# zhykoties/Multi-Head-Recommendation-with-Human-Priors

Hardware: AMD Instinct MI355X
Metric: user-sequences/sec/node (HSTU Pixel8M, seqlen 200) (higher is better)
Workload: dtype bf16; 1 GPU; cfg1: HSTU Pixel8M-shaped train step, L=200 P=8 D=256 8 layers x 8 heads, 4 prior heads, N=453938 items, 8192 negatives/pool, B=128/GPU, loss=prior, bf16-mixed, fused AdamW over all parameters (item table: lazy replay of gradient-free steps, flushed inside the timed region); step replayed from a hipGraph; encoder on packed rows (the loader's row capacity, one step graph per capacity); global_batch=128, seq_len=200, parallelism=dp1

## Files before the change

### include/mhr.h

```cpp
#ifndef MHR_H
#define MHR_H

#include <stdint.h>

#ifdef __cplusplus
extern "C" {
#endif

#define MHR_F32 0
#define MHR_BF16 1

#define MHR_OK 0
#define MHR_EINVAL (-1)
#define MHR_ELAUNCH (-2)

const char* mhr_last_error(void);
int mhr_abi_version(void);


int mhr_bad_id_count(int64_t* host_count, int reset);

int mhr_embedding_gather_fwd(const float* table, int64_t n_rows, int dim,
                             const int64_t* ids, int64_t n_ids,
                             void* out, int out_dtype,
                             const float* pos_table, int seq_len, int window_len,
                             void* x_out, int x_dtype, int64_t n_x_ids, void* stream);

int mhr_embedding_gather_step(const float* table, int64_t n_rows, int dim, const int64_t* ids, int64_t n_ids,
                              int64_t n_item_ids, float* rows_out, const float* pos_table, int seq_len, int window_len,
                              float* x_out, void* neg_out, float* neg_norms, const int32_t* row_of, const int32_t* src_of,
                              int capacity, void* stream);

int mhr_embedding_scatter_add_bwd(const void* grad_rows, int grad_dtype, const int64_t* ids, int64_t n_ids,
                                  float* grad_table, int64_t n_rows, int dim, void* stream);

int mhr_sparse_rows_segment_sum(const int64_t* sorted_ids, const int64_t* perm, int64_t n_ids,
                                const void* grad_a, int a_dtype, int64_t n_a,
                                const void* grad_b, int b_dtype, int64_t n_b,
                                const float* x_grad, int seq_len, int window_len, const int32_t* x_row_of,
                                float* out_rows, int32_t* row_slot, int64_t n_rows, int dim, void* stream);

int mhr_pos_grad_packed(const float* d_x, const int32_t* row_of, int B, int L, int dim, float* out, void* stream);
int mhr_window_rows_add_packed(const float* rows, int64_t n_rows, int window_len, int seq_len, const float* d_x,
                               const int32_t* row_of, int dim, float* out, void* stream);

int mhr_adam_rows(float* w, float* m, float* v, int64_t n_rows, int dim,
                  const float* grad_rows, int32_t* row_slot, float grad_scale,
                  float lr, float beta1, float beta2, float eps, float weight_decay, int step, void* stream);

int mhr_adam_flat(float* w, const float* g, float* m, float* v, int64_t n, float grad_scale,
                  float lr, float beta1, float beta2, float eps, float weight_decay, int step, void* w_bf16,
                  const float* hist, int hist_len, const int64_t* step_dev, void* stream);
int mhr_adam_consts(float lr, float beta1, float beta2, float eps, float weight_decay, int step, float* out4);
int mhr_adam_rows_lazy(float* w, float* m, float* v, int64_t n_rows, int dim, const int64_t* ids, int64_t n_ids,
                       const float* grad_rows, int32_t* row_slot, int32_t* last_step, const float* hist,
                       int hist_len, int step, float grad_scale, float beta1, float beta2, float eps, int mode,
                       const int64_t* step_dev, void* stream);

int mhr_sum_rows_into(const void* x_bf16, int64_t rows, int64_t cols, float* out, void* stream);
int mhr_sum_rows_f32_into(const float* x, int64_t rows, int64_t cols, float* out, void* stream);
int mhr_sum_rows_many(const int64_t* ptrs, int n, int64_t rows, int64_t cols, void* stream);


int mhr_layernorm_fwd(const void* x, int x_dtype, void* y, int y_dtype, float* mean, float* rstd,
                      int64_t rows, int dim, float eps, void* stream);
int mhr_layernorm_bwd(const void* dy, int dy_dtype, const void* x, int x_dtype, const float* mean, const float* rstd,
                      void* dx, int dx_dtype, int accumulate, int64_t rows, int dim, void* stream);
int mhr_add_cast(const float* x, const void* y_bf16, float* out, void* out_bf16, int64_t n, void* stream);

int mhr_add_layernorm_fwd(const float* x, const void* y_bf16, float* x_out, void* xn_bf16, float* mean, float* rstd,
                          int64_t rows, int dim, float eps, const int32_t* first_row, int seq_len, void* stream);
int mhr_add_layernorm_bwd(const void* d_xn_bf16, const float* x_out, const float* mean, const float* rstd,
                          const float* d_xout, float* dx, void* dy_bf16, int64_t rows, int dim,
                          const int32_t* first_row, int seq_len, void* stream);

int mhr_ln_gate_fwd(const void* u_base, int64_t u_stride, const void* a, int dtype, void* o, int o_dtype,
                    float* mean, float* rstd, int64_t rows, int dim, float eps,
                    float dropout_p, uint64_t seed, const int64_t* step_seed,
                    const int32_t* first_row, int seq_len, void* stream);
int mhr_ln_gate_bwd(const void* d_o, int do_dtype, const void* u_base, int64_t u_stride, const void* a, int dtype,
                    const float* mean, const float* rstd, void* du_base, int64_t du_stride, void* da,
                    int64_t rows, int dim, float dropout_p, uint64_t seed, const int64_t* step_seed,
                    const int32_t* first_row, int seq_len, void* stream);

int mhr_l2norm_rows(const void* x, int x_dtype, void* y, int y_dtype, float* norms, int64_t rows, int dim, void* stream);
int mhr_l2norm_rows_bwd(const float* dy, const float* x, const float* norms, float* dx, int64_t rows, int dim, void* stream);
int mhr_l2norm_rows_indexed_bwd(const float* dy, const float* table, int64_t n_src_rows, const int64_t* ids, const float* norms,
                                float* dx, int64_t rows, int dim, void* stream);

int mhr_hstu_attn_fwd(const void* q, const void* k, const void* v, int64_t row_stride,
                      const uint8_t* key_valid, void* out,
                      void* act_q, void* act_k, void* act_v, int64_t act_stride,
                      int B, int L, int n_heads, int head_dim, int apply_silu, void* stream);
int mhr_hstu_attn_bwd(const void* q_pre, const void* k_pre, const void* v_pre, int64_t row_stride,
                      const void* act_q, const void* act_k, const void* act_v, int64_t act_stride,
                      const uint8_t* key_valid, const void* d_out,
                      void* dq, void* dk, void* dv, int64_t d_stride,
                      int B, int L, int n_heads, int head_dim, int apply_silu, void* stream);

int mhr_rows_gemm_supported(int M, int N, int K, int w_is_kn);
int mhr_rows_gemm(const void* a, int64_t lda, const void* w, int64_t ldw, int w_is_kn, const void* bias,
                  void* c, int64_t ldc, int M, int N, int K, void* stream);

int mhr_attn_seq_layout(const uint8_t* key_valid, int B, int L, int32_t* first_block, int32_t* seq_order,
                        int32_t* first_row , void* stream);
int mhr_hstu_attn_fwd_seq(const void* q, const void* k, const void* v, int64_t row_stride,
                          const uint8_t* key_valid, void* out,
                          void* act_q, void* act_k, void* act_v, int64_t act_stride,
                          int B, int L, int n_heads, int head_dim, int apply_silu,
                          const int32_t* first_block, const int32_t* seq_order, const int32_t* cu_rows, int n_rows_total,
                          void* stream);
int mhr_hstu_attn_bwd_seq(const void* q_pre, const void* k_pre, const void* v_pre, int64_t row_stride,
                          const void* act_q, const void* act_k, const void* act_v, int64_t act_stride,
                          const uint8_t* key_valid, const void* d_out,
                          void* dq, void* dk, void* dv, int64_t d_stride,
                          int B, int L, int n_heads, int head_dim, int apply_silu,
                          const int32_t* first_block, const int32_t* seq_order, const int32_t* cu_rows, int n_rows_total,
                          void* stream);

int mhr_seq_pack_maps(const uint8_t* key_valid, int B, int L, int capacity, int32_t* cu_rows, int32_t* src_of, int32_t* row_of,
                      int32_t* overflow, void* stream);
int mhr_seq_pack_maps_guarded(const uint8_t* key_valid, int B, int L, int capacity, int32_t* cu_rows, int32_t* src_of,
                              int32_t* row_of, int32_t* overflow, int32_t* guard, void* stream);
int mhr_rows_gather_masked(const void* src, int dtype, const int32_t* idx, void* out, int64_t n_out, int dim, void* stream);


int mhr_rmsnorm_fwd(const float* x, const void* res_bf16, const float* weight, float* x_out, void* y_bf16, float* rstd,
                    int64_t rows, int dim, float eps, void* stream);
int mhr_rmsnorm_bwd_parts(int64_t rows);
int mhr_rmsnorm_bwd(const void* dy_bf16, const float* x_out, const float* weight, const float* rstd, const float* d_xout,
                    float* dx, void* dres_bf16, float* dw_part, int64_t rows, int dim, void* stream);

int mhr_swiglu_fwd(const void* gate_up_bf16, void* act_bf16, int64_t rows, int ffn, void* stream);
int mhr_swiglu_bwd(const void* gate_up_bf16, const void* d_act_bf16, void* d_gate_up_bf16, int64_t rows, int ffn, void* stream);

int mhr_rope_inplace(void* x_bf16, int64_t row_stride, const int32_t* positions, const float* cos_table,
                     const float* sin_table, int64_t n_tokens, int seq_len, int n_heads, int head_dim, int max_pos,
                     int inverse, void* stream);

int mhr_softmax_attn_fwd(const void* q, const void* k, const void* v, int64_t row_stride, const int32_t* cu_seqlens,
                         const uint8_t* key_valid, void* out, float* lse, int n_seqs, int max_len, int n_heads,
                         int n_kv_heads, int head_dim, float scale, void* stream);
int mhr_softmax_attn_bwd(const void* q, const void* k, const void* v, int64_t row_stride, const int32_t* cu_seqlens,
                         const uint8_t* key_valid, const void* out, const void* d_out, const float* lse, void* dq,
                         int64_t dq_stride, void* dk, void* dv, int64_t dkv_stride, int n_seqs, int max_len, int n_heads,
                         int n_kv_heads, int head_dim, float scale, void* stream);

int mhr_token_compact(const uint8_t* mask, const int32_t* q_all, const int32_t* p_all, const int32_t* o_all,
                      int n_groups, int n_slots, int tok_cap, int32_t* q_idx, int32_t* p_idx, int32_t* o_idx,
                      int32_t* n_tok, int32_t* scratch, int32_t* tok_of_slot, const int32_t* row_of, int seq_len,
                      int n_heads, int head_stride, void* stream);

int mhr_heads_residual_fwd(const float* x, const void* z_bf16, float* out, int64_t n_tok, int seq_len, int n_heads,
                           int dim, void* stream);
int mhr_heads_residual_bwd(const float* d_out, const void* z_bf16, void* dz_bf16, float* dx, int64_t n_tok,
                           int seq_len, int n_heads, int dim, void* stream);

int mhr_row_maps(const int32_t* q_idx, const int32_t* n_tok_dev, int n_groups, int tok_cap, int row_cap,
                 int32_t* row_q, int32_t* row_first, int32_t* tok2row, int32_t* n_row, int32_t* scratch, void* stream);

int mhr_nce_log_counters(const int32_t* n_valid, const int32_t* rank, const int32_t* o_idx, const int32_t* n_tok_dev,
                         int group, int tok_cap, const int32_t* ks_host, int n_k, uint64_t* scratch8, float* out, void* stream);

int mhr_loss_reduce(const float* bucket_sum, const float* bucket_cnt, const float* weight, int n_groups, int n_buckets,
                    int n_segments, float* total, float* out, void* stream);
int mhr_loss_reduce_bwd(const float* d_total, const float* bucket_cnt, const float* weight, int n, float* w_out, void* stream);

int mhr_nce_fwd(const void* q_rows, const int32_t* q_idx, const void* p_rows, const int32_t* p_idx, int io_dtype,
                const void* negs, int n_neg, int dim, int n_groups, const int32_t* n_tok_dev, int tok_cap,
                const float* logit_scale_dev, float thres,
                float* sum_out, int32_t* n_valid, int32_t* rank,
                void* qn_out, void* pn_out, uint32_t* supp_out, float* q_inv, float* p_inv, float* s_pos,
                int log_group, float* u_out, int64_t n_p_rows, uint32_t* fix_words, const int32_t* fix_row_list,
                const int32_t* fix_n_rows, int32_t* fix_slot_of_row, void* stream);
int mhr_nce_finalize(const float* sum, const float* s_pos, int n_groups, const int32_t* n_tok_dev, int tok_cap,
                     const float* logit_scale_dev, float* loss, float* lse, int32_t* n_valid,
                     const int32_t* bucket_idx, int n_buckets, float* bucket_sum, float* bucket_cnt, void* stream);
int mhr_nce_bwd_tokens(const void* qn, const void* pn, const float* u, int dim, int n_groups,
                       const int32_t* n_tok_dev, int tok_cap, const float* logit_scale_dev,
                       const float* lse, const float* w, const float* q_inv, const float* p_inv, const float* s_pos,
                       const int32_t* q_idx, const int32_t* p_idx,
                       float* dq_rows, float* dp_rows, float* d_logit_scale, float* lw_out,
                       const int32_t* w_bucket, int n_buckets, int64_t* dq_fix, int64_t* dp_fix,
                       float* dls_part, void* stream);
int mhr_nce_bwd_negs(const void* qn, const void* negs, const uint32_t* supp, int n_neg, int dim, int n_groups,
// ... 145 lines not shown
```

### multi-head-recommendation-with-human-priors_amd/code/REC/model/hstu_functional.py

```python
import os
from collections import OrderedDict

import torch
from torch.autograd import Function

from mhr_amd import ops

_SPLITK_MAX = int(os.environ.get("MHR_SPLITK_MAX", "16"))
_SUM_KERNEL = os.environ.get("MHR_SUM_KERNEL", "1") != "0"


class LayerNormFn(Function):

    @staticmethod
    def forward(ctx, x, eps, out=None):
        y, mean, rstd = ops.layernorm_fwd(x, torch.bfloat16, eps, out=out)
        ctx.save_for_backward(x, mean, rstd)
        return y

    @staticmethod
    def backward(ctx, dy):
        x, mean, rstd = ctx.saved_tensors
        return ops.layernorm_bwd(dy.contiguous(), x, mean, rstd, dx_dtype=torch.float32), None, None

# ... 31 lines not shown
    @staticmethod
    def backward(ctx, d_xout, d_xn):
        x_out, mean, rstd = ctx.saved_tensors
        if d_xout is None:
            d_xout = torch.zeros_like(x_out)
        if d_xn is None:
            d_xn = torch.zeros(x_out.shape, dtype=torch.bfloat16, device=x_out.device)
        dx, dy = ops.add_layernorm_bwd(d_xn.contiguous(), x_out, mean, rstd, d_xout.contiguous().float(), dy_out=ctx.dy_out,
                                       dead=ctx.dead)
        return dx, dy, None, None, None, None


class AddCastFn(Function):

    @staticmethod
    def forward(ctx, x, y, dy_out=None):
        ctx.dy_out = dy_out
        return ops.add_cast(x.contiguous(), y.contiguous())

    @staticmethod
    def backward(ctx, d_out, d_out16):
        if d_out is None and d_out16 is None:
            return None, None, None
        if d_out16 is None:
            return d_out, d_out.to(torch.bfloat16), None
        if d_out is None:
            return d_out16.float(), d_out16, None
        return ops.add_cast(d_out.contiguous(), d_out16.contiguous(), out16=ctx.dy_out) + (None,)


class WeightGradStack:

    def __init__(self, opt, uvqk_params, o_params, R, D, device):
        L = len(uvqk_params)
        self.opt, self.L, self.R, self.D = opt, L, R, D
        self.params = {"uvqk": list(uvqk_params), "o": list(o_params)}
        bf = dict(dtype=torch.bfloat16, device=device)
        self.xn, self.dh = torch.empty(L, R, D, **bf), torch.empty(L, R, 4 * D, **bf)
        self.o, self.dy = torch.empty(L, R, D, **bf), torch.empty(L, R, D, **bf)
        self.seen = {"uvqk": set(), "o": set()}
        opt.defer(self.flush)

    def operands(self, kind, layer, x, dy):
        xs, ds = (self.xn, self.dh) if kind == "uvqk" else (self.o, self.dy)
        if x.data_ptr() != xs[layer].data_ptr():
            xs[layer].copy_(x.reshape(xs[layer].shape))
        if dy.data_ptr() != ds[layer].data_ptr():
            ds[layer].copy_(dy.reshape(ds[layer].shape))
        self.seen[kind].add(layer)

    @staticmethod
    def _splits(R, prefer):
        return next((s for s in prefer if R % s == 0 and R // s >= 256), 1)

    def flush(self):
        n = {k: len(v) for k, v in self.seen.items()}
        if n["uvqk"] == 0 and n["o"] == 0:
            return
        if n["uvqk"] != self.L or n["o"] != self.L:
            raise RuntimeError(f"WeightGradStack: {n} of {self.L} layers handed their operands over")
        L, R, D = self.L, self.R, self.D
        S1 = self._splits(R, (8, 4, 2))
        w1 = torch.bmm(self.xn.view(L * S1, R // S1, D).transpose(1, 2), self.dh.view(L * S1, R // S1, 4 * D))
        S2 = self._splits(R, (16, 8, 4, 2))
        w2 = torch.bmm(self.dy.view(L * S2, R // S2, D).transpose(1, 2), self.o.view(L * S2, R // S2, D))
        for l in range(L):
            self.opt.queue_rows_sum(w1[l * S1:(l + 1) * S1].view(S1, -1), self.params["uvqk"][l].grad)
            self.opt.queue_rows_sum(w2[l * S2:(l + 1) * S2].view(S2, -1), self.params["o"][l].grad)
        self.seen = {"uvqk": set(), "o": set()}


ROWS_GEMM = os.environ.get("MHR_ROWS_GEMM", "1") != "0"
ROWS_GEMM_MIN_M = int(os.environ.get("MHR_ROWS_GEMM_MIN_M", "8192"))


def _rows_gemm_pays(x, w_kn):
    M, K = x.shape
    N = w_kn.shape[1]
    return (K == 256 and N >= 1024 and M >= ROWS_GEMM_MIN_M and x.dtype == torch.bfloat16 and w_kn.dtype == torch.bfloat16
            and x.stride(1) == 1 and w_kn.is_contiguous() and x.stride(0) % 8 == 0 and x.data_ptr() % 16 == 0 and w_kn.data_ptr() % 16 == 0
            and ops.rows_gemm_supported(M, N, K, True))


class SplitKLinearFn(Function):

    @staticmethod
    def forward(ctx, x, w, b, w_is_nk, w_bf16, defer=None):
        ctx.defer = defer
        if w_bf16 is None:
            sh = getattr(w, "_mhr_bf16", None)
            w_bf16 = sh if (sh is not None and w._version == w._mhr_ver) else None
        wb = w.to(torch.bfloat16) if w_bf16 is None else w_bf16
        bb = None
        if b is not None:
            sh = getattr(b, "_mhr_bf16", None)
            bb = sh if (sh is not None and b._version == b._mhr_ver) else b.to(torch.bfloat16)
        if w_is_nk:
            y = torch.nn.functional.linear(x, wb, bb)
        elif ROWS_GEMM and _rows_gemm_pays(x, wb):
            y = ops.rows_gemm(x, wb, None, w_is_kn=True)
        else:
            y = x @ wb
        ctx.save_for_backward(x, wb)
        ctx.w_is_nk, ctx.has_bias = w_is_nk, b is not None
        ctx.w_leaf = w if getattr(w, "_mhr_direct_grad", False) and w.grad is not None else None
        ctx.b_leaf = b if (b is not None and getattr(b, "_mhr_direct_grad", False) and b.grad is not None) else None
        return y

    @staticmethod
    def _into(leaf, parts):
        g = leaf.grad
        if _SUM_KERNEL and parts.dtype == torch.bfloat16 and parts.is_contiguous() and g.is_contiguous() and g.numel() % 8 == 0:
            ops.sum_rows_into(parts, g)
        else:
            g.add_(torch.sum(parts, 0, dtype=torch.float32).view_as(g))

    @staticmethod
    def backward(ctx, dy):
        x, wb = ctx.saved_tensors
        dy = dy.contiguous()
        dx = dy @ wb if ctx.w_is_nk else dy @ wb.t()
        R = x.shape[0]
        if ctx.defer is not None and ctx.w_leaf is not None:
            stack, kind, layer = ctx.defer
            stack.operands(kind, layer, x, dy)
            if ctx.has_bias and ctx.b_leaf is not None:
                bopt = getattr(ctx.b_leaf, "_mhr_opt", None)
                if not (bopt is not None and bopt.queue_bias_sum(dy, ctx.b_leaf)):
                    SplitKLinearFn._into(ctx.b_leaf, dy)
                return dx, None, None, None, None, None
            return dx, None, (torch.sum(dy, 0, dtype=torch.float32) if ctx.has_bias else None), None, None, None
        tiles = -(-wb.shape[0] // 256) * -(-wb.shape[1] // 256)
        s_max = min(max(1, 256 // tiles), _SPLITK_MAX)
        S = next((s for s in (64, 32, 16, 8, 4, 2) if s <= s_max and R % s == 0 and R // s >= 256), 1)
        xs, dys = x.view(S, R // S, -1), dy.view(S, R // S, -1)
        opt = getattr(ctx.w_leaf, "_mhr_opt", None) if ctx.w_leaf is not None else None
        slot = opt.partial_view(ctx.w_leaf, S) if (opt is not None and S > 1 and _SUM_KERNEL) else None
        if ctx.w_is_nk:
            dw = torch.bmm(dys.transpose(1, 2), xs, out=slot) if slot is not None else torch.bmm(dys.transpose(1, 2), xs)
        else:
            dw = torch.bmm(xs.transpose(1, 2), dys, out=slot) if slot is not None else torch.bmm(xs.transpose(1, 2), dys)
        if slot is not None:
            dw = None
        elif ctx.w_leaf is not None:
            SplitKLinearFn._into(ctx.w_leaf, dw)
            dw = None
        else:
            dw = torch.sum(dw, 0, dtype=torch.float32) if S > 1 else dw[0].float()
        db = None
        if ctx.has_bias:
            if ctx.b_leaf is not None:
                bopt = getattr(ctx.b_leaf, "_mhr_opt", None)
                if not (bopt is not None and _SUM_KERNEL and bopt.queue_bias_sum(dy, ctx.b_leaf)):
                    SplitKLinearFn._into(ctx.b_leaf, dy)
            else:
                db = torch.sum(dy, 0, dtype=torch.float32)
        return dx, dw, db, None, None, None


class FusedHeadsLinearFn(Function):

    @staticmethod
    def forward(ctx, x, w16, b16, gw, gb):
        ctx.save_for_backward(x, w16)
        ctx.gw, ctx.gb = gw, gb
        return torch.nn.functional.linear(x, w16, b16)

    @staticmethod
    def backward(ctx, dy):
        x, w16 = ctx.saved_tensors
        dy = dy.contiguous()
        dx = dy @ w16
        R = x.shape[0]
        tiles = -(-w16.shape[0] // 256) * -(-w16.shape[1] // 256)
        s_max = min(max(1, 256 // tiles), _SPLITK_MAX)
        S = next((s for s in (64, 32, 16, 8, 4, 2) if s <= s_max and R % s == 0 and R // s >= 256), 1)
        dw = torch.bmm(dy.view(S, R // S, -1).transpose(1, 2), x.view(S, R // S, -1))
        ops.sum_rows_into(dw, ctx.gw)
        ops.sum_rows_into(dy, ctx.gb)
        return dx, None, None, None, None


class HeadsResidualFn(Function):

    @staticmethod
    def forward(ctx, x, z, B, L, H):
        ctx.save_for_backward(z)
        ctx.cfg = (B, L, H)
        return ops.heads_residual_fwd(x.contiguous(), z.contiguous(), B, L, H)

    @staticmethod
    def backward(ctx, d_out):
        (z,) = ctx.saved_tensors
        B, L, H = ctx.cfg
        dz, dx = ops.heads_residual_bwd(d_out.contiguous().float(), z, B, L, H)
        return dx, dz, None, None, None


class FusedParamLinearFn(Function):

    @staticmethod
    def forward(ctx, x, w16, gview, leaf):
        ctx.save_for_backward(x, w16)
        ctx.gview, ctx.leaf = gview, leaf
        return torch.nn.functional.linear(x, w16)

    @staticmethod
    def backward(ctx, dy):
        from mhr_amd import optim
        x, w16 = ctx.saved_tensors
        dy = dy.contiguous()
        dx = dy @ w16
        dw = torch.mm(dy.t(), x, out_dtype=torch.float32)
        if getattr(ctx.leaf, "_mhr_epoch_f", -1) != optim.GRAD_EPOCH:
            ctx.leaf._mhr_epoch_f = optim.GRAD_EPOCH
            ctx.gview.copy_(dw)
        else:
            ctx.gview.add_(dw)
        return dx, None, None, None


class MoveRowsFn(Function):

    @staticmethod
    def forward(ctx, x, fwd_idx, bwd_idx):
        ctx.bwd_idx = bwd_idx
        return ops.rows_gather_masked(x.contiguous(), fwd_idx)

    @staticmethod
    def backward(ctx, dy):
        return ops.rows_gather_masked(dy.contiguous(), ctx.bwd_idx), None, None


class HSTUCoreFn(Function):

    @staticmethod
    def forward(ctx, h, key_valid, B, L, n_heads, head_dim, eps, dropout_p, seed, seed_dev=None, o_out=None, dh_out=None):
        D = n_heads * head_dim
        layout = getattr(key_valid, "_mhr_layout", None)
        a, _ = ops.hstu_attn_fwd(h, key_valid, B, L, n_heads, head_dim, apply_silu=True, save_act=False, layout=layout)
        dead = (layout[2], L) if (ops.DEAD_ROWS and layout is not None and len(layout) > 2 and layout[2] is not None
                                  and getattr(key_valid, "_mhr_dead_ok", True)) else None
        o, mean, rstd = ops.ln_gate_fwd(h, a, D, torch.bfloat16, eps, dropout_p, seed, seed_dev, out=o_out, dead=dead)
        ctx.dh_out = dh_out
        ctx.save_for_backward(h, key_valid, a, mean, rstd)
        ctx.cfg = (B, L, n_heads, head_dim, dropout_p, seed, seed_dev)
        ctx.layout, ctx.dead = layout, dead
        return o

    @staticmethod
    def backward(ctx, d_o):
        h, key_valid, a, mean, rstd = ctx.saved_tensors
        B, L, n_heads, head_dim, dropout_p, seed, seed_dev = ctx.cfg
        D = n_heads * head_dim
        dh = torch.empty_like(h) if ctx.dh_out is None else ctx.dh_out.view(h.shape)
# ... 294 lines not shown
```

### multi-head-recommendation-with-human-priors_amd/csrc/rows_gemm.hip

```cpp
#include <algorithm>

#include "stream_gemm.h"

namespace {

typedef unsigned u32x2_t __attribute__((ext_vector_type(2)));

#ifdef RGX_STAMP
__device__ unsigned long long g_rg_stamps[4096 * 4];
#define RG_STAMP(k)                                                                     \
  {                                                                                     \
    __builtin_amdgcn_sched_barrier(0);                                                  \
    unsigned long long t_;                                                              \
    asm volatile("s_memtime %0\n\ts_waitcnt lgkmcnt(0)" : "=s"(t_)::"memory");          \
    __builtin_amdgcn_sched_barrier(0);                                                  \
    if (threadIdx.x == 0 && blockIdx.x < 4096) g_rg_stamps[blockIdx.x * 4 + (k)] = t_;  \
  }
#define RG_PHASE(k)                                                                     \
  {                                                                                     \
    __builtin_amdgcn_sched_barrier(0);                                                  \
    unsigned long long t_;                                                              \
    asm volatile("s_memtime %0\n\ts_waitcnt lgkmcnt(0)" : "=s"(t_)::"memory");          \
    __builtin_amdgcn_sched_barrier(0);                                                  \
    pacc_[k] += t_ - ph_;                                                               \
// ... 127 lines not shown
    } else {
      dp.template piece<k>(tiles + slot * T::BYTES, reinterpret_cast<const char*>(A) + (int64_t)tn * T::BYTES);
    }
  };
  auto dma_tile = [&](auto slot_c, int tn) {
    auto f = [&](auto k_c) { dma_piece(slot_c, k_c, tn); };
    sg::static_for<P::PW>(f);
  };
  sg::RowAddr<NKS> ra;
  ra.init(la, tiles);

  const int n_lane = n_wave + 8 * half;
  const bool full_cols = n_wave + 64 <= N;

  const int n_loc = t1 - t0, t_last = t1 - 1;
  dma_tile(std::integral_constant<int, 0>{}, t0);
  dma_tile(std::integral_constant<int, 1>{}, min(t0 + 1, t_last));
#ifdef RGX_STAMP
  unsigned long long ph_ = 0, pacc_[8] = {0, 0, 0, 0, 0, 0, 0, 0};
  RG_PHASE(7)
#endif
  sg::u32x4 o[RF][2];
  auto store_piece = [&](auto idx_c, int ts, bool all) {
    constexpr int idx = decltype(idx_c)::value, f = idx >> 1, gp = idx & 1;
    bf16_t* p = C + (int64_t)(ts * 32 + r) * ldc + n_lane + f * 32 + gp * 16;
    if (all || (ts * 32 + r < M && n_lane + f * 32 + gp * 16 < N)) *reinterpret_cast<sg::u32x4*>(p) = o[f][gp];
  };
  constexpr int NOPS = P::PW + 4;
  sg::ring_loop<3>(n_loc, [&](auto slot_c, int i) {
    constexpr int cur = decltype(slot_c)::value, nxt = (cur + 2) % 3;
    const int t = t0 + i;
    RG_PHASE(0)
    if (i > 2 && full_cols) sg::wait_vmcnt<P::PW + 8>();
    else if (i == 2 && full_cols) sg::wait_vmcnt<P::PW + 4>();
    else sg::wait_vmcnt<P::PW>();
    sg::ring_barrier();
    RG_PHASE(1)
    f32x16 acc[RF];
#pragma unroll
    for (int f = 0; f < RF; ++f) {
      if constexpr (HAS_BIAS) acc[f] = acc0[f];
      else acc[f] = sg::zero16();
    }
    const int t_dma = min(t + 2, t_last);
    const bool st_all = full_cols;
    mma_tile_gaps<NKS, RF, cur * T::BYTES>(ra, frag, acc, [&](auto ks_c) {
      constexpr int ks = decltype(ks_c)::value;
      auto op = [&](auto j_c) {
        constexpr int jj = decltype(j_c)::value;
        if constexpr (jj * NKS / NOPS == ks) {
          if constexpr (jj < P::PW) dma_piece(std::integral_constant<int, nxt>{}, j_c, t_dma);
          else if (i > 0) store_piece(std::integral_constant<int, jj - P::PW>{}, t - 1, st_all);
        }
      };
      sg::static_for<NOPS>(op);
    });
    RG_PHASE(3)
#pragma unroll
    for (int f = 0; f < RF; ++f) {
#pragma unroll
      for (int gp = 0; gp < 2; ++gp) {
        const int gx = 8 * gp, gy = 8 * gp + 4;
        const uint32_t x0 = sg::cvt_pk_bf16(acc[f][gx + 0], acc[f][gx + 1]), x1 = sg::cvt_pk_bf16(acc[f][gx + 2], acc[f][gx + 3]);
        const uint32_t y0 = sg::cvt_pk_bf16(acc[f][gy + 0], acc[f][gy + 1]), y1 = sg::cvt_pk_bf16(acc[f][gy + 2], acc[f][gy + 3]);
        const u32x2_t s0 = __builtin_amdgcn_permlane32_swap(x0, y0, false, false);
        const u32x2_t s1 = __builtin_amdgcn_permlane32_swap(x1, y1, false, false);
        o[f][gp] = sg::u32x4{s0.x, s1.x, s0.y, s1.y};
      }
    }
    RG_PHASE(4)
  });
  {
    const bool all = full_cols && t_last * 32 + 32 <= M;
    auto st = [&](auto idx_c) { store_piece(idx_c, t_last, all); };
    sg::static_for<4>(st);
  }
  RG_STAMP(2)
#ifdef RGX_STAMP
  if (threadIdx.x == 0 && blockIdx.x == 37)
    for (int k = 0; k < 7; ++k) g_rg_stamps[4096 * 4 - 8 + k] += pacc_[k];
#endif
  sg::wait_vmcnt<0>();
  RG_STAMP(3)
}

}

#ifdef RGX_STAMP
extern "C" int mhr_debug_read_rg_stamps(unsigned long long* host, int n) {
  return (int)hipMemcpyFromSymbol(host, HIP_SYMBOL(g_rg_stamps), (size_t)n * sizeof(unsigned long long));
}
#endif

extern "C" int mhr_rows_gemm_supported(int M, int N, int K, int w_is_kn) {
  return (K == 64 || K == 128 || K == 256) && N > 0 && N % (w_is_kn ? 256 : 8) == 0 && M > 0;
}

extern "C" int mhr_rows_gemm(const void* a, int64_t lda, const void* w, int64_t ldw, int w_is_kn, const void* bias, void* c,
                             int64_t ldc, int M, int N, int K, void* stream) {
  MHR_REQUIRE(a && w && c, "rows_gemm: null pointer");
  MHR_REQUIRE(mhr_rows_gemm_supported(M, N, K, w_is_kn),
              "rows_gemm: M=%d N=%d K=%d unsupported (K in {64, 128, 256}; N a multiple of 8, of 256 with W stored [K, N])", M, N, K);
  MHR_REQUIRE(lda >= K && ldw >= (w_is_kn ? N : K) && ldc >= N && lda % 8 == 0 && ldw % 8 == 0 && ldc % 8 == 0,
              "rows_gemm: leading dimensions must cover the rows and be multiples of 8 elements");
  MHR_REQUIRE(((uintptr_t)a | (uintptr_t)w | (uintptr_t)c) % 16 == 0, "rows_gemm: operands must be 16-byte aligned");
  const int n_tiles = (M + 31) / 32;
  const int n_cg = (N + 255) / 256;
  int n_streams = (512 / n_cg) & ~7;
  while (n_streams > 8 && n_tiles / n_streams < 3) n_streams -= 8;
  if (n_streams < 8) n_streams = 8;
  const bool strided = lda != K || M % 32 != 0;
  const int nks = K / 16;
  size_t lds = 4 * (size_t)(32 * K * 2);
  if (w_is_kn) lds = std::max(lds, (size_t)std::min(K / 32, 4) * 16384);
  hipStream_t s = (hipStream_t)stream;
#define L____(NKS, ST, HB, KN)                                                                                            \
  hipLaunchKernelGGL((rows_gemm_kernel<NKS, ST, HB, KN>), dim3(n_cg * n_streams), dim3(256), lds, s, (const bf16_t*)a, lda, \
                     (const bf16_t*)w, ldw, (const bf16_t*)bias, (bf16_t*)c, ldc, M, N, n_tiles, n_cg, n_streams)
#define L___(NKS, ST, HB)                    \
  if (w_is_kn) { L____(NKS, ST, HB, true); } \
  else { L____(NKS, ST, HB, false); }
#define L__(NKS, ST)                \
  if (bias) { L___(NKS, ST, true) } \
  else { L___(NKS, ST, false) }
#define L_(NKS)                     \
  if (strided) { L__(NKS, true) }   \
  else { L__(NKS, false) }
  if (nks == 16) { L_(16) }
  else if (nks == 8) { L_(8) }
  else { L_(4) }
#undef L_
#undef L__
#undef L___
#undef L____
  MHR_CHECK_LAUNCH("rows_gemm");
  return MHR_OK;
}
```

### multi-head-recommendation-with-human-priors_amd/ops.py

```python
import os

import torch

from . import lib

F32, BF16 = lib.F32, lib.BF16

PROFILE = None


def _timed_call(name, *args):
    if PROFILE is not None and name in PROFILE:
        e0, e1 = torch.cuda.Event(enable_timing=True), torch.cuda.Event(enable_timing=True)
        e0.record()
        lib.call(name, *args)
        e1.record()
        PROFILE[name].append((e0, e1))
    else:
        lib.call(name, *args)


def profile_summary(with_max=False):
    out = {}
    for name, evs in (PROFILE or {}).items():
# ... 281 lines not shown
             rstd.data_ptr(), dh.data_ptr(), dh.stride(0), da.data_ptr(), rows, dim, dropout_p, seed, _ptr(seed_dev),
             *_dead_args(dead, rows), _stream())
    return da


def l2norm_rows(x, out_dtype=torch.bfloat16, want_norms=False):
    _chk(x, "x")
    D = x.shape[-1]
    rows = x.numel() // D
    y = torch.empty(x.shape, dtype=out_dtype, device=x.device)
    norms = torch.empty(rows, dtype=torch.float32, device=x.device) if want_norms else None
    lib.call("mhr_l2norm_rows", x.data_ptr(), _dt(x), y.data_ptr(), _dt(y), _ptr(norms), rows, D, _stream())
    return (y, norms) if want_norms else y


def l2norm_rows_bwd(dy, x, norms):
    _chk(dy, "dy", torch.float32)
    _chk(x, "x", torch.float32)
    D = x.shape[-1]
    dx = torch.empty_like(x)
    lib.call("mhr_l2norm_rows_bwd", dy.data_ptr(), x.data_ptr(), norms.data_ptr(), dx.data_ptr(), x.numel() // D, D, _stream())
    return dx


def embedding_gather_step(table, pos_table, ids_all, n_item_ids, seq_len, window, pack=None):
    _chk(table, "table", torch.float32)
    _chk(pos_table, "pos_table", torch.float32)
    _chk(ids_all, "ids_all", torch.int64)
    D = table.shape[1]
    dev = table.device
    n = ids_all.numel()
    n_neg = n - n_item_ids
    rows = torch.empty(n_item_ids, D, dtype=torch.float32, device=dev)
    row_of = src_of = None
    cap = 0
    if pack is not None:
        row_of, src_of, cap = pack
        _chk(row_of, "row_of", torch.int32)
        _chk(src_of, "src_of", torch.int32)
        cap = int(cap)
        assert row_of.numel() == n_item_ids // window * seq_len and src_of.numel() == cap
        x = torch.empty(cap, D, dtype=torch.float32, device=dev)
    else:
        x = torch.empty(n_item_ids // window, seq_len, D, dtype=torch.float32, device=dev)
    negs = torch.empty(n_neg, D, dtype=torch.bfloat16, device=dev)
    norms = torch.empty(n_neg, dtype=torch.float32, device=dev)
    _timed_call("mhr_embedding_gather_step", table.data_ptr(), table.shape[0], D, ids_all.data_ptr(), n, n_item_ids, rows.data_ptr(),
                pos_table.data_ptr(), seq_len, window, x.data_ptr(), negs.data_ptr(), norms.data_ptr(), _ptr(row_of), _ptr(src_of),
                cap, _stream())
    return rows, x, negs, norms


def l2norm_rows_indexed_bwd(dy, table, ids, norms):
    _chk(dy, "dy", torch.float32)
    _chk(table, "table", torch.float32)
    _chk(ids, "ids", torch.int64)
    D = table.shape[1]
    dx = torch.empty(ids.numel(), D, dtype=torch.float32, device=table.device)
    lib.call("mhr_l2norm_rows_indexed_bwd", dy.data_ptr(), table.data_ptr(), table.shape[0], ids.data_ptr(), norms.data_ptr(),
             dx.data_ptr(), ids.numel(), D, _stream())
    return dx


def rows_gemm_supported(M, N, K, w_is_kn=False):
    return K in (64, 128, 256) and N > 0 and N % (256 if w_is_kn else 8) == 0 and M > 0


def rows_gemm(a, w, bias=None, out=None, w_is_kn=False):
    for t_, nm in ((a, "a"), (w, "w")):
        if not (t_.is_cuda and t_.dtype == torch.bfloat16 and t_.dim() == 2 and t_.stride(1) == 1):
            raise ValueError(f"rows_gemm: {nm} must be a 2-d bf16 device tensor with unit inner stride")
    M, K = a.shape
    N = w.shape[1] if w_is_kn else w.shape[0]
    if (w.shape[0] if w_is_kn else w.shape[1]) != K:
        raise ValueError("rows_gemm: inner dimensions differ")
    if out is None:
        out = torch.empty(M, N, dtype=torch.bfloat16, device=a.device)
    elif out.shape != (M, N) or out.dtype != torch.bfloat16 or out.stride(1) != 1:
        raise ValueError("rows_gemm: out must be [M, N] bf16 with unit inner stride")
    if bias is not None:
        _chk(bias, "bias", torch.bfloat16)
    _timed_call("mhr_rows_gemm", a.data_ptr(), a.stride(0), w.data_ptr(), w.stride(0), 1 if w_is_kn else 0,
                bias.data_ptr() if bias is not None else 0, out.data_ptr(), out.stride(0), M, N, K, _stream())
    return out


def seq_pack_maps(key_valid, B, L, capacity, guard=None):
    _chk(key_valid, "key_valid", torch.uint8)
    dev = key_valid.device
    cu = torch.empty(B + 1, dtype=torch.int32, device=dev)
    src_of = torch.empty(capacity, dtype=torch.int32, device=dev)
    row_of = torch.empty(B * L, dtype=torch.int32, device=dev)
    overflow = torch.empty(1, dtype=torch.int32, device=dev)
    if guard is None:
        lib.call("mhr_seq_pack_maps", key_valid.data_ptr(), B, L, int(capacity), cu.data_ptr(), src_of.data_ptr(), row_of.data_ptr(),
                 overflow.data_ptr(), _stream())
    else:
        _chk(guard, "guard", torch.int32)
        if guard.numel() != 4 or guard.device != dev:
            raise ValueError("seq_pack_maps: guard must be int32 [4] on the mask's device")
        lib.call("mhr_seq_pack_maps_guarded", key_valid.data_ptr(), B, L, int(capacity), cu.data_ptr(), src_of.data_ptr(),
                 row_of.data_ptr(), overflow.data_ptr(), guard.data_ptr(), _stream())
    return cu, src_of, row_of, overflow


def rows_gather_masked(src, idx, out=None):
    _chk(src, "src")
    _chk(idx, "idx", torch.int32)
    n, dim = idx.numel(), src.shape[-1]
    if out is None:
        out = torch.empty(n, dim, dtype=src.dtype, device=src.device)
    lib.call("mhr_rows_gather_masked", src.data_ptr(), _dt(src), idx.data_ptr(), out.data_ptr(), n, dim, _stream())
    return out


PACK_ROWS = os.environ.get("MHR_PACK_ROWS", "1") != "0"
PACK_HEADS = os.environ.get("MHR_PACK_HEADS", "1") != "0"
DEAD_ROWS = os.environ.get("MHR_DEAD_ROWS", "1") != "0"
SEQ_LAYOUT = os.environ.get("MHR_ATTN_SEQ_LAYOUT", "1") != "0"


def attn_seq_layout(key_valid, B, L, order=True):
    _chk(key_valid, "key_valid", torch.uint8)
    first = torch.empty(B, dtype=torch.int32, device=key_valid.device)
    first_row = torch.empty(B, dtype=torch.int32, device=key_valid.device)
    order_t = torch.empty(B, dtype=torch.int32, device=key_valid.device) if order else None
    lib.call("mhr_attn_seq_layout", key_valid.data_ptr(), B, L, first.data_ptr(), order_t.data_ptr() if order else 0,
             first_row.data_ptr(), _stream())
    return first, order_t, first_row


def _layout_ptrs(layout):
    if layout is None:
        return 0, 0, 0
    first, order = layout[0], layout[1]
    cu = layout[3] if len(layout) > 3 else None
    return (first.data_ptr() if first is not None else 0), (order.data_ptr() if order is not None else 0), (cu.data_ptr() if cu is not None else 0)


def hstu_attn_fwd(h, key_valid, B, L, n_heads, head_dim, apply_silu=True, save_act=True, layout=None):
    _chk(h, "h", torch.bfloat16)
    _chk(key_valid, "key_valid", torch.uint8)
    D = n_heads * head_dim
    stride = h.stride(0)
    esz = 2
    base = h.data_ptr()
    v_ptr, q_ptr, k_ptr = base + D * esz, base + 2 * D * esz, base + 3 * D * esz
    R = h.shape[0]
    out = torch.empty(R, D, dtype=torch.bfloat16, device=h.device)
    act = torch.empty(R, 3 * D, dtype=torch.bfloat16, device=h.device) if save_act else None
    aq = act.data_ptr() if save_act else 0
    fb, so, cu = _layout_ptrs(layout)
    _timed_call("mhr_hstu_attn_fwd_seq", q_ptr, k_ptr, v_ptr, stride, key_valid.data_ptr(), out.data_ptr(),
             aq, aq + D * esz if save_act else 0, aq + 2 * D * esz if save_act else 0, 3 * D,
             B, L, n_heads, head_dim, 1 if apply_silu else 0, fb, so, cu, R if cu else 0, _stream())
    return out, act


def hstu_attn_bwd(h, act, key_valid, d_out, dh, B, L, n_heads, head_dim, apply_silu=True, layout=None):
    D = n_heads * head_dim
    esz = 2
    base, dbase = h.data_ptr(), dh.data_ptr()
    abase = act.data_ptr() if act is not None else 0
    fb, so, cu = _layout_ptrs(layout)
    _timed_call("mhr_hstu_attn_bwd_seq", base + 2 * D * esz, base + 3 * D * esz, base + D * esz, h.stride(0),
             abase, abase + D * esz if act is not None else 0, abase + 2 * D * esz if act is not None else 0,
# ... 842 lines not shown
```

Baseline: 33990 seq/s.

## Add deep-K rows GEMM kernel for linear input-gradient in backward

```diff
diff --git a/include/mhr.h b/include/mhr.h
--- a/include/mhr.h
+++ b/include/mhr.h
@@ -101,6 +101,10 @@
 int mhr_rows_gemm_supported(int M, int N, int K, int w_is_kn);
 int mhr_rows_gemm(const void* a, int64_t lda, const void* w, int64_t ldw, int w_is_kn, const void* bias,
                   void* c, int64_t ldc, int M, int N, int K, void* stream);
+
+int mhr_rows_gemm_deep_supported(int M, int N, int K, int w_is_kn);
+int mhr_rows_gemm_deep(const void* a, int64_t lda, const void* w, int64_t ldw, int w_is_kn,
+                       void* c, int64_t ldc, int M, int N, int K, void* stream);
 
 int mhr_attn_seq_layout(const uint8_t* key_valid, int B, int L, int32_t* first_block, int32_t* seq_order,
                         int32_t* first_row , void* stream);
diff --git a/multi-head-recommendation-with-human-priors_amd/code/REC/model/hstu_functional.py b/multi-head-recommendation-with-human-priors_amd/code/REC/model/hstu_functional.py
--- a/multi-head-recommendation-with-human-priors_amd/code/REC/model/hstu_functional.py
+++ b/multi-head-recommendation-with-human-priors_amd/code/REC/model/hstu_functional.py
@@ -137,6 +137,25 @@
             and ops.rows_gemm_supported(M, N, K, True))
 
 
+ROWS_GEMM_DEEP = os.environ.get("MHR_ROWS_GEMM_DEEP", "1") != "0"
+ROWS_GEMM_DEEP_MIN_M = int(os.environ.get("MHR_ROWS_GEMM_DEEP_MIN_M", "16384"))
+ROWS_GEMM_DEEP_MAX_M = int(os.environ.get("MHR_ROWS_GEMM_DEEP_MAX_M", "18432"))
+
+
+def _rows_gemm_deep_pays(dy, w, w_is_kn):
+    M, K = dy.shape
+    N = w.shape[1] if w_is_kn else w.shape[0]
+    return (ROWS_GEMM_DEEP and ROWS_GEMM_DEEP_MIN_M <= M <= ROWS_GEMM_DEEP_MAX_M and dy.dtype == torch.bfloat16 and w.dtype == torch.bfloat16
+            and dy.is_contiguous() and w.dim() == 2 and w.stride(1) == 1 and w.stride(0) % 8 == 0
+            and dy.data_ptr() % 16 == 0 and w.data_ptr() % 16 == 0 and ops.rows_gemm_deep_supported(M, N, K, w_is_kn))
+
+
+def _input_grad(dy, w, w_is_kn):
+    if _rows_gemm_deep_pays(dy, w, w_is_kn):
+        return ops.rows_gemm_deep(dy, w, w_is_kn=w_is_kn)
+    return dy @ w if w_is_kn else dy @ w.t()
+
+
 class SplitKLinearFn(Function):
 
     @staticmethod
@@ -174,7 +193,7 @@
     def backward(ctx, dy):
         x, wb = ctx.saved_tensors
         dy = dy.contiguous()
-        dx = dy @ wb if ctx.w_is_nk else dy @ wb.t()
+        dx = _input_grad(dy, wb, ctx.w_is_nk)
         R = x.shape[0]
         if ctx.defer is not None and ctx.w_leaf is not None:
             stack, kind, layer = ctx.defer
@@ -225,7 +244,7 @@
     def backward(ctx, dy):
         x, w16 = ctx.saved_tensors
         dy = dy.contiguous()
-        dx = dy @ w16
+        dx = _input_grad(dy, w16, True)
         R = x.shape[0]
         tiles = -(-w16.shape[0] // 256) * -(-w16.shape[1] // 256)
         s_max = min(max(1, 256 // tiles), _SPLITK_MAX)
diff --git a/multi-head-recommendation-with-human-priors_amd/csrc/rows_gemm.hip b/multi-head-recommendation-with-human-priors_amd/csrc/rows_gemm.hip
--- a/multi-head-recommendation-with-human-priors_amd/csrc/rows_gemm.hip
+++ b/multi-head-recommendation-with-human-priors_amd/csrc/rows_gemm.hip
@@ -233,6 +233,165 @@
 #endif
   sg::wait_vmcnt<0>();
   RG_STAMP(3)
+}
+
+template <bool W_KN, bool PARTIAL>
+__global__ __launch_bounds__(256, 1) void rows_gemm_deep_kernel(const bf16_t* __restrict__ A, int64_t lda, const bf16_t* __restrict__ W,
+                                                                int64_t ldw, bf16_t* __restrict__ C, int64_t ldc, int M, int n_tiles,
+                                                                int n_cg, int n_streams) {
+  using T = sg::Tile<16>;
+  using TW = sg::Tile<8>;
+  constexpr int NC = 4;
+  extern __shared__ __attribute__((aligned(16))) unsigned char smem[];
+  unsigned char* ring = smem;
+  unsigned char* stg = smem + NC * T::BYTES;
+
+  const int w = blockIdx.x, xcd = w & 7, j = w >> 3;
+  const int cg = j % n_cg, stream = (j / n_cg) * 8 + xcd;
+  const int t0 = (int)((int64_t)stream * n_tiles / n_streams), t1 = (int)((int64_t)(stream + 1) * n_tiles / n_streams);
+  if (t0 >= t1) return;
+  const int wave = threadIdx.x >> 6, lane = threadIdx.x & 63, r = lane & 31, half = lane >> 5;
+  const int wv = __builtin_amdgcn_readfirstlane(wave);
+  const int n_wave = cg * 128 + wv * 32;
+  const int t_last = t1 - 1;
+
+  using P = sg::DmaPieces<16>;
+  P dp;
+  dp.init(wv, lane, (int)(lda * 2));
+  auto dma_piece = [&](auto slot_c, auto k_c, int tn) {
+    constexpr int slot = decltype(slot_c)::value, k = decltype(k_c)::value;
+    if constexpr (PARTIAL) {
+      dp.template piece_rows<k>(ring + slot * T::BYTES, [=](int rr) {
+        const int m = tn * 32 + rr;
+        return A + (int64_t)(m < M ? m : M - 1) * lda + slot * 256;
+      }, lane);
+    } else {
+      dp.template piece<k>(ring + slot * T::BYTES, reinterpret_cast<const char*>(A + (int64_t)tn * 32 * lda + slot * 256));
+    }
+  };
+  auto dma_chunk = [&](auto slot_c, int tn) {
+    auto f = [&](auto k_c) { dma_piece(slot_c, k_c, tn); };
+    sg::static_for<P::PW>(f);
+  };
+  dma_chunk(std::integral_constant<int, 0>{}, t0);
+  dma_chunk(std::integral_constant<int, 1>{}, t0);
+  dma_chunk(std::integral_constant<int, 2>{}, t0);
+
+  bf16x8 frag[NC][1][16];
+  if constexpr (!W_KN) {
+    using TQ = sg::Tile<4>;
+    constexpr int NB = 6, NR = 16;
+    sg::LaneAddr<4> lw;
+    lw.init(lane);
+    unsigned char* my = stg + wv * 5 * TQ::BYTES;
+    unsigned char* my5 = ring + 3 * T::BYTES + wv * TQ::BYTES;
+    const uint32_t my_addr = sg::lds_addr(my), my5_addr = sg::lds_addr(my5);
+    const int slot = lane & 7;
+    const bf16_t* wrow = W + (int64_t)(n_wave + (lane >> 3)) * ldw;
+    auto w_issue = [&](auto rd_c) {
+      constexpr int rd = decltype(rd_c)::value, b = rd % NB;
+      unsigned char* img = b < 5 ? my + b * TQ::BYTES : my5;
+#pragma unroll
+      for (int pc = 0; pc < 4; ++pc) {
+        const int row = pc * 8 + (lane >> 3);
+        const bf16_t* src = wrow + (int64_t)(pc * 8) * ldw + rd * 64 + ((slot ^ TQ::key(row)) << 3);
+        __builtin_amdgcn_global_load_lds((sg::gptr_t)src, (sg::lptr_t)(img + pc * 1024), 16, 0, 0);
+      }
+    };
+    sg::static_for<NB>(w_issue);
+    auto w_round = [&](auto rd_c) {
+      constexpr int rd = decltype(rd_c)::value, b = rd % NB;
+      constexpr int younger = (NR - 1 - rd) < NB - 1 ? (NR - 1 - rd) : NB - 1;
+      sg::wait_vmcnt<4 * younger>();
+      const uint32_t base = b < 5 ? my_addr + b * TQ::BYTES : my5_addr;
+      sg::u32x4 v[4];
+#pragma unroll
+      for (int ks = 0; ks < 4; ++ks) v[ks] = sg::ds_read_b128_asm<0>(base + (uint32_t)lw.a[ks]);
+      sg::wait_lgkm_values<0>(v[0], v[1], v[2], v[3]);
+#pragma unroll
+      for (int ks = 0; ks < 4; ++ks) frag[rd >> 2][0][(rd & 3) * 4 + ks] = __builtin_bit_cast(bf16x8, v[ks]);
+      asm volatile("" ::: "memory");
+      __builtin_amdgcn_sched_barrier(0);
+      if constexpr (rd + NB < NR) w_issue(std::integral_constant<int, rd + NB>{});
+    };
+    sg::static_for<NR>(w_round);
+  } else {
+    typedef __attribute__((address_space(3))) bf16x4 lds_bf16x4;
+    sg::LaneAddr<8> lw;
+    lw.init(lane);
+    const int tr0 = wv == 0 ? lw.t[0][0] : wv == 1 ? lw.t[0][1] : wv == 2 ? lw.t[0][2] : lw.t[0][3];
+    const int tr1 = wv == 0 ? lw.t[1][0] : wv == 1 ? lw.t[1][1] : wv == 2 ? lw.t[1][2] : lw.t[1][3];
+#pragma unroll
+    for (int rd = 0; rd < 4; ++rd) {
+      if (rd) __syncthreads();
+#pragma unroll
+      for (int q = 0; q < 8; ++q) {
+        const int k0 = (rd * 8 + q) * 32;
+        sg::Dma<8>::issue(stg + q * TW::BYTES, [=](int rr) { return W + (int64_t)(k0 + rr) * ldw + cg * 128; }, wv, lane);
+      }
+      sg::wait_vmcnt<0>();
+      __syncthreads();
+#pragma unroll
+      for (int q = 0; q < 8; ++q) {
+#pragma unroll
+        for (int s2 = 0; s2 < 2; ++s2) {
+          const unsigned char* base = stg + q * TW::BYTES + 16 * s2 * TW::ROW_BYTES;
+          const bf16x4 lo = __builtin_amdgcn_ds_read_tr16_b64_v4bf16((lds_bf16x4*)(base + tr0));
+          const bf16x4 hi = __builtin_amdgcn_ds_read_tr16_b64_v4bf16((lds_bf16x4*)(base + tr1));
+          const u32x2_t l2 = __builtin_bit_cast(u32x2_t, lo), h2 = __builtin_bit_cast(u32x2_t, hi);
+          const u32x2_t s0 = __builtin_amdgcn_permlane32_swap(l2.x, h2.x, false, false);
+          const u32x2_t s1 = __builtin_amdgcn_permlane32_swap(l2.y, h2.y, false, false);
+          frag[rd][0][q * 2 + s2] = __builtin_bit_cast(bf16x8, sg::u32x4{s0.x, s1.x, s0.y, s1.y});
+        }
+      }
+    }
+  }
+
+  sg::LaneAddr<16> la;
+  la.init(lane);
+  sg::RowAddr<16> ra;
+  ra.init(la, ring);
+  const int n_lane = n_wave + 8 * half;
+  sg::u32x4 o[2];
+  auto store_piece = [&](auto gp_c, int ts, bool all) {
+    constexpr int gp = decltype(gp_c)::value;
+    bf16_t* p = C + (int64_t)(ts * 32 + r) * ldc + n_lane + gp * 16;
+    if (all || ts * 32 + r < M) *reinterpret_cast<sg::u32x4*>(p) = o[gp];
+  };
+  f32x16 acc[1];
+  acc[0] = sg::zero16();
+  sg::ring_loop<NC>(NC * (t1 - t0), [&](auto slot_c, int i) {
+    constexpr int cur = decltype(slot_c)::value, nxt = (cur + 3) % NC;
+    const int t = t0 + (i >> 2);
+    sg::wait_vmcnt<2 * P::PW>();
+    sg::ring_barrier();
+    if constexpr (cur == 0) acc[0] = sg::zero16();
+    const int t_dma = min(t + (cur >= 1 ? 1 : 0), t_last);
+    mma_tile_gaps<16, 1, cur * T::BYTES>(ra, frag[cur], acc, [&](auto ks_c) {
+      constexpr int ks = decltype(ks_c)::value;
+      if constexpr (ks % 4 == 0) dma_piece(std::integral_constant<int, nxt>{}, std::integral_constant<int, ks / 4>{}, t_dma);
+      if constexpr (cur == 0 && (ks == 2 || ks == 6)) {
+        if (i > 0) store_piece(std::integral_constant<int, (ks - 2) / 4>{}, t - 1, true);
+      }
+    });
+    if constexpr (cur == NC - 1) {
+#pragma unroll
+      for (int gp = 0; gp < 2; ++gp) {
+        const int gx = 8 * gp, gy = 8 * gp + 4;
+        const uint32_t x0 = sg::cvt_pk_bf16(acc[0][gx + 0], acc[0][gx + 1]), x1 = sg::cvt_pk_bf16(acc[0][gx + 2], acc[0][gx + 3]);
+        const uint32_t y0 = sg::cvt_pk_bf16(acc[0][gy + 0], acc[0][gy + 1]), y1 = sg::cvt_pk_bf16(acc[0][gy + 2], acc[0][gy + 3]);
+        const u32x2_t s0 = __builtin_amdgcn_permlane32_swap(x0, y0, false, false);
+        const u32x2_t s1 = __builtin_amdgcn_permlane32_swap(x1, y1, false, false);
+        o[gp] = sg::u32x4{s0.x, s1.x, s0.y, s1.y};
+      }
+    }
+  });
+  {
+    const bool all = t_last * 32 + 32 <= M;
+    auto st = [&](auto gp_c) { store_piece(gp_c, t_last, all); };
+    sg::static_for<2>(st);
+  }
+  sg::wait_vmcnt<0>();
 }
 
 }
@@ -287,3 +446,41 @@
   MHR_CHECK_LAUNCH("rows_gemm");
   return MHR_OK;
 }
+
+extern "C" int mhr_rows_gemm_deep_supported(int M, int N, int K, int w_is_kn) {
+  (void)w_is_kn;
+  return K == 1024 && N > 0 && N % 128 == 0 && M > 0;
+}
+
+extern "C" int mhr_rows_gemm_deep(const void* a, int64_t lda, const void* w, int64_t ldw, int w_is_kn, void* c, int64_t ldc, int M,
+                                  int N, int K, void* stream) {
+  MHR_REQUIRE(a && w && c, "rows_gemm_deep: null pointer");
+  MHR_REQUIRE(mhr_rows_gemm_deep_supported(M, N, K, w_is_kn),
+              "rows_gemm_deep: M=%d N=%d K=%d unsupported (K = 1024; N a multiple of 128)", M, N, K);
+  MHR_REQUIRE(lda >= K && ldw >= (w_is_kn ? N : K) && ldc >= N && lda % 8 == 0 && ldw % 8 == 0 && ldc % 8 == 0 && lda <= (1 << 24),
+              "rows_gemm_deep: leading dimensions must cover the rows and be multiples of 8 elements (lda at most 2^24)");
+  MHR_REQUIRE(((uintptr_t)a | (uintptr_t)w | (uintptr_t)c) % 16 == 0, "rows_gemm_deep: operands must be 16-byte aligned");
+  const int n_tiles = (M + 31) / 32;
+  const int n_cg = N / 128;
+  int n_streams = (256 / n_cg) & ~7;
+  while (n_streams > 8 && n_tiles / n_streams < 2) n_streams -= 8;
+  if (n_streams < 8) n_streams = 8;
+  const bool partial = M % 32 != 0;
+  const size_t lds = 4 * (size_t)16384 + 20 * (size_t)4096;
+  hipStream_t s = (hipStream_t)stream;
+#define L_(KN, PT)                                                                                                            \
+  {                                                                                                                           \
+    auto kern = rows_gemm_deep_kernel<KN, PT>;                                                                                \
+    (void)hipFuncSetAttribute((const void*)kern, hipFuncAttributeMaxDynamicSharedMemorySize, (int)lds);                       \
+    hipLaunchKernelGGL(kern, dim3(n_cg * n_streams), dim3(256), lds, s, (const bf16_t*)a, lda, (const bf16_t*)w, ldw,          \
+                       (bf16_t*)c, ldc, M, n_tiles, n_cg, n_streams);                                                         \
+  }
+  if (w_is_kn) {
+    if (partial) L_(true, true) else L_(true, false)
+  } else {
+    if (partial) L_(false, true) else L_(false, false)
+  }
+#undef L_
+  MHR_CHECK_LAUNCH("rows_gemm_deep");
+  return MHR_OK;
+}
diff --git a/multi-head-recommendation-with-human-priors_amd/ops.py b/multi-head-recommendation-with-human-priors_amd/ops.py
--- a/multi-head-recommendation-with-human-priors_amd/ops.py
+++ b/multi-head-recommendation-with-human-priors_amd/ops.py
@@ -387,6 +387,27 @@
         _chk(bias, "bias", torch.bfloat16)
     _timed_call("mhr_rows_gemm", a.data_ptr(), a.stride(0), w.data_ptr(), w.stride(0), 1 if w_is_kn else 0,
                 bias.data_ptr() if bias is not None else 0, out.data_ptr(), out.stride(0), M, N, K, _stream())
+    return out
+
+
+def rows_gemm_deep_supported(M, N, K, w_is_kn=False):
+    return K == 1024 and N > 0 and N % 128 == 0 and M > 0
+
+
+def rows_gemm_deep(a, w, out=None, w_is_kn=False):
+    for t_, nm in ((a, "a"), (w, "w")):
+        if not (t_.is_cuda and t_.dtype == torch.bfloat16 and t_.dim() == 2 and t_.stride(1) == 1):
+            raise ValueError(f"rows_gemm_deep: {nm} must be a 2-d bf16 device tensor with unit inner stride")
+    M, K = a.shape
+    N = w.shape[1] if w_is_kn else w.shape[0]
+    if (w.shape[0] if w_is_kn else w.shape[1]) != K:
+        raise ValueError("rows_gemm_deep: inner dimensions differ")
+    if out is None:
+        out = torch.empty(M, N, dtype=torch.bfloat16, device=a.device)
+    elif out.shape != (M, N) or out.dtype != torch.bfloat16 or out.stride(1) != 1:
+        raise ValueError("rows_gemm_deep: out must be [M, N] bf16 with unit inner stride")
+    _timed_call("mhr_rows_gemm_deep", a.data_ptr(), a.stride(0), w.data_ptr(), w.stride(0), 1 if w_is_kn else 0,
+                out.data_ptr(), out.stride(0), M, N, K, _stream())
     return out
 
 
```

Measured after the change: 34450 seq/s, median of 6. 1.4% higher.
